# lrjconan/LanczosNetwork

Measured on AMD Instinct MI355X. Metric: molecules/sec LanczosNet forward, QM8 batch=1024, higher is better.
Workload: dtype f32; 1 GPU; QM8 LanczosNet batch=1024/GPU, N<=32 dense L (tile N=26), K=20, fp32, 7x128 layers, 1xMI355X per rank; step = [pack L + batch plan + Lanczos + tridiagonal eigensolver (Ritz pairs)] (one launch) + spectral gains + fused forward; global_batch=1024, parallelism=dp1 (batch shards, async score all-gather per step)

## Files before the change

include/lanczosnet_hip.h:

```cpp
#ifndef LANCZOSNET_HIP_H_
#define LANCZOSNET_HIP_H_

#include <stdint.h>

#ifdef __cplusplus
extern "C" {
#endif

#define LNZ_ABI_VERSION 7
#define LNZ_OK 0
#define LNZ_EINVAL (-1)
#define LNZ_ELAUNCH (-2)
#define LNZ_ENOTSUP (-3)

#define LNZ_TILE 32
#define LNZ_MAX_CHANNELS 32
#define LNZ_STRIP_SUB 6
#define LNZ_STRIP_INTS 80
#define LNZ_STRIP_MAX_B 2048
#define LNZ_RARE_DEBUG_INTS 512

typedef void* lnz_stream_t;

int lnz_abi_version(void);
// ... 154 lines not shown
int lnz_pack_rows_k8(const float* W, int rows, int cols, int64_t ld, float* Wp,
                     lnz_stream_t stream);
int lnz_pack_rows_k8_split(const float* W, int rows, int cols, int64_t ld, float* Wp,
                           lnz_stream_t stream);
int64_t lnz_pack_fold_weights_size(int num_layer, int din0, int dhid);
int lnz_pack_fold_weights(const float* Wp, const int64_t* w_off_host, int num_layer, int din0, int dhid,
                          int n_short, int n_long, int n_edge, float* Wf, lnz_stream_t stream);
int lnz_pack_bias_rows(const float* bias, int rows, float* bp, lnz_stream_t stream);
int lnz_pack_laplacian(const float* L, int64_t stride_b, int64_t stride_r, int64_t stride_c,
                       int64_t stride_ch, int B, int N, int C, float* Lp, lnz_stream_t stream);
int lnz_pack_laplacian_ident(const float* L, int64_t stride_b, int64_t stride_r, int64_t stride_c,
                             int64_t stride_ch, int B, int N, int C, float* Lp, uint32_t* ident,
                             lnz_stream_t stream);

int64_t lnz_spectral_mlp_pack_size(int S);
int lnz_pack_spectral_mlp(const float* W0, const float* b0, const float* W2, const float* b2,
                          const float* W4, const float* b4, const float* W6, const float* b6,
                          int S, float* pack, lnz_stream_t stream);
int lnz_pack_spectral_mlp_layers(const float* const* ptrs, int num_layer, int S, float* pack,
                                 lnz_stream_t stream);
int lnz_spectral_gains(const float* D, int B, int K, const int32_t* dist_host, int S,
                       int num_layer, int kind, const float* mlp_pack, float* G,
                       lnz_stream_t stream);
int lnz_spectral_gains_rows(const float* D, int B, int K, const int32_t* dist_host, int S,
                            int num_layer, int kind, const float* mlp_pack, const int32_t* rows,
                            const int32_t* n_rows, float* G, lnz_stream_t stream);

int lnz_spectral_mlp_grad_floats(int S);
int lnz_spectral_mlp_grad_parts(int n_rows_max, int num_layer, int n_cu);
int lnz_spectral_mlp_grad(const float* D, int B, int K, const int32_t* dist_host, int S,
// ... 266 lines not shown
```

lanczosnet_amd/_lib.py:

```python
import ctypes as C
import os

_HERE = os.path.dirname(os.path.abspath(__file__))
LIB_PATH = os.environ.get('LANCZOSNET_HIP_LIB') or os.path.join(_HERE, 'csrc', 'liblanczosnet_hip.so')

LNZ_OK, LNZ_EINVAL, LNZ_ELAUNCH, LNZ_ENOTSUP = 0, -1, -2, -3
ABI_VERSION = 7


class LnzError(RuntimeError):
  def __init__(self, code, msg):
    super().__init__('lanczosnet_hip error %d: %s' % (code, msg))
    self.code = code


class NotSupported(LnzError, NotImplementedError):
  pass


class ForwardArgs(C.Structure):
  _fields_ = [
      ('B', C.c_int32), ('N', C.c_int32), ('K', C.c_int32),
      ('num_layer', C.c_int32),
      ('din0', C.c_int32), ('dhid', C.c_int32), ('dout', C.c_int32),
# ... 91 lines not shown
    'lnz_pack_fold_weights_size': (C.c_int64, [_I, _I, _I]),
    'lnz_pack_fold_weights': (C.c_int, [_P, C.POINTER(C.c_int64), _I, _I, _I, _I, _I, _I, _P, _P]),
    'lnz_pack_bias_rows': (C.c_int, [_P, _I, _P, _P]),
    'lnz_pack_laplacian': (C.c_int, [_P, _L, _L, _L, _L, _I, _I, _I, _P, _P]),
    'lnz_collate_qm8': (C.c_int, [_P, _P, _P, _P, _P, _P, _L, _I, _I, _I, _I, _P, _P, _P, _P, _P, _P]),
    'lnz_plan_wg_cap': (C.c_int, [_I, _I]),
    'lnz_pack_laplacian_plan': (C.c_int, [_P, _L, _L, _L, _L, _I, _I, _I, _P, _P, _I, _I, _P, _P, _I, _P, _P, _P, _P, _P, _P]),
    'lnz_pack_laplacian_ident': (C.c_int, [_P, _L, _L, _L, _L, _I, _I, _I, _P, _P, _P]),
    'lnz_prepare_batch_prev_gains': (C.c_int, [_P, _L, _L, _L, _L, _I, _I, _I, _P, _P, _P, _I, _I, _P, _P, _I, _P, _P, _P, _P, _P, _P, _I, _P, _P, C.POINTER(C.c_int32), _I, _I, _P, _P, _P, _P, _P]),
    'lnz_prepare_batch': (C.c_int, [_P, _L, _L, _L, _L, _I, _I, _I, _P, _P, _P, _I, _I, _P, _P, _I, _P, _P, _P, _P, _P, _P, _P, _P, _P]),
    'lnz_plan_batch': (C.c_int, [_P, _I, _I, _I, _I, _P, _P, _I, _P, _P, _P, _P, _P]),
    'lnz_plan_strips': (C.c_int, [_P, _I, _I, _I, _P, _P, _P]),
    'lnz_strip_cap': (C.c_int, [_I]),
    'lnz_plan_tiles': (C.c_int, [_P, _I, _I, _I, _I, _P, _P, _P]),
    'lnz_spectral_mlp_pack_size': (C.c_int64, [_I]),
    'lnz_pack_spectral_mlp': (C.c_int, [_P] * 8 + [_I, _P, _P]),
    'lnz_pack_spectral_mlp_layers': (C.c_int, [_P, _I, _I, _P, _P]),
    'lnz_spectral_mlp_grad_parts': (C.c_int, [_I, _I, _I]),
    'lnz_spectral_gains_rows_split': (C.c_int, [_P, _I, _I, _P, _I, _I, _I, _P, _P, _P, _P, _P, _L, _P]),
    'lnz_spectral_gains_rows_split_to': (C.c_int, [_P, _I, _I, _P, _I, _I, _I, _P, _P, _P, _P, _P, _P, _L, _P]),
    'lnz_split_laplacian_pack': (C.c_int, [_P, _L, _P]),
    'lnz_split_laplacian_pack_to': (C.c_int, [_P, _L, _P, _P]),
    'lnz_spectral_mlp_grad_floats': (C.c_int, [_I]),
    'lnz_embedding_grad': (C.c_int, [_P, _I, _I, _P, _L, _L, _I, _I, _I, _P, _P]),
    'lnz_spectral_mlp_grad': (C.c_int, [_P, _I, _I, _P, _I, _I, _P, _P, _P, _P, _I, _P, _P]),
    'lnz_spectral_gains': (C.c_int, [_P, _I, _I, C.POINTER(C.c_int32), _I, _I, _I, _P, _P, _P]),
    'lnz_spectral_gains_rows': (C.c_int, [_P, _I, _I, C.POINTER(C.c_int32), _I, _I, _I, _P, _P, _P, _P, _P]),
    'lnz_lanczosnet_input_grad': (C.c_int, [C.POINTER(ForwardArgs), _P]),
    'lnz_lanczosnet_messages': (C.c_int, [C.POINTER(ForwardArgs), _P]),
    'lnz_lanczosnet_gain_grad': (C.c_int, [C.POINTER(ForwardArgs), _P]),
# ... 87 lines not shown
```

lanczosnet_amd/csrc/gains_body.hpp:

```cpp
#pragma once
#include "common.hpp"

namespace lnz_gains {

constexpr int HID = 128;
constexpr int HT = HID / 32;
constexpr int SMAX = 16;
constexpr int OFF_W0 = 0;
constexpr int OFF_B0 = OFF_W0 + HT * 8 * 64;
constexpr int OFF_B2 = OFF_B0 + HT * 1024;
constexpr int OFF_B4 = OFF_B2 + HT * 1024;
constexpr int OFF_B6 = OFF_B4 + HT * 1024;
constexpr int OFF_W2 = OFF_B6 + 1024;
constexpr int OFF_W4 = OFF_W2 + HT * 16 * 256;
constexpr int OFF_W6 = OFF_W4 + HT * 16 * 256;
#ifndef LNZ_GAINS_RING
#define LNZ_GAINS_RING 8
#endif
#ifndef LNZ_GAINS_DIST
#define LNZ_GAINS_DIST (LNZ_GAINS_RING - 2)
#endif
constexpr int RING = LNZ_GAINS_RING;
constexpr int PACK_SIZE = OFF_W6 + 16 * 256 + RING * 256;
constexpr int NSTEP = 2 * HT * 16 + 16;

struct DistArr {
  int32_t v[SMAX];
};

__device__ inline float powi(float x, int p) {
  double base = (double)x, acc = 1.0;
  int e = p < 0 ? -p : p;
  while (e) {
    if (e & 1) acc *= base;
    base *= base;
    e >>= 1;
  }
  return (float)(p < 0 ? 1.0 / acc : acc);
}

__device__ inline f32x16 load_bias_frag(const float* __restrict__ bp, int lane) {
  const float4* p = reinterpret_cast<const float4*>(bp) + lane * 4;
  f32x16 acc;
// ... 39 lines not shown
#pragma unroll
    for (int t = 0; t < RT; ++t) acc1[t] = lnz::mfma32(a.y, Hin[t][ti][4 * g + 1], acc1[t]);
#pragma unroll
    for (int t = 0; t < RT; ++t) acc[t] = lnz::mfma32(a.z, Hin[t][ti][4 * g + 2], acc[t]);
#pragma unroll
    for (int t = 0; t < RT; ++t) acc1[t] = lnz::mfma32(a.w, Hin[t][ti][4 * g + 3], acc1[t]);
    __builtin_amdgcn_sched_barrier(0);
  }
#pragma unroll
  for (int t = 0; t < RT; ++t) {
#pragma unroll
    for (int i = 0; i < 16; ++i) res[t][i] = acc[t][i] + acc1[t][i];
  }
}

template <int RT>
__device__ __forceinline__ void gains_mlp_tiles(const float* __restrict__ D, const int (&row)[RT],
                                                const bool (&valid)[RT], const int l,
                                                const int lane, int B, int K, const DistArr& dist,
                                                int S, const float* __restrict__ mlp_pack,
                                                float* __restrict__ G) {
  const int hh = lane >> 5;
  const float* pk = mlp_pack + (int64_t)l * PACK_SIZE;
#ifdef LNZ_GAINS_PROBE_STAGGER
  for (int i = 0; i < (int)((blockIdx.x & (LNZ_GAINS_PROBE_STAGGER_N - 1)) * LNZ_GAINS_PROBE_STAGGER); ++i)
    __builtin_amdgcn_s_sleep(16);
#endif

  const float4* __restrict__ wstream = reinterpret_cast<const float4*>(pk + OFF_W2) + lane;
  float4 ring[RING];
#pragma unroll
  for (int f = 0; f < LNZ_GAINS_DIST; ++f) ring[f] = wstream[f * 64];

  const int steps0 = S < 8 ? S : 8;
  f32x16 h1[RT][HT], h2[RT][HT];
  {
    float w0[HT][8];
#pragma unroll
    for (int ot = 0; ot < HT; ++ot) {
#pragma unroll
      for (int t = 0; t < 8; ++t) w0[ot][t] = pk[OFF_W0 + (ot * 8 + t) * 64 + lane];
    }
#pragma unroll
    for (int rt = 0; rt < RT; ++rt) {
      const float dval = valid[rt] ? D[row[rt]] : 0.0f;
      float feat[8];
#pragma unroll
      for (int t = 0; t < 8; ++t) {
#ifdef LNZ_GAINS_PROBE_NOPOW
        float lo = t < S ? dval : 0.0f;
        float hi = (8 + t) < S ? dval : 0.0f;
// ... 16 lines not shown
  }
  f32x16 res[RT];
#define LNZ_DENSE(F0, IN, OUT, OT, BOFF)                                   \
  {                                                                        \
    const f32x16 bb = load_bias_frag(pk + (BOFF), lane);                   \
    dense_tile<F0, RT>(wstream, ring, IN, res);                            \
    _Pragma("unroll") for (int rt = 0; rt < RT; ++rt) OUT[rt][OT] = relu_bias16(res[rt], bb); \
  }
  LNZ_DENSE(0, h1, h2, 0, OFF_B2 + 0 * 1024)
  LNZ_DENSE(16, h1, h2, 1, OFF_B2 + 1 * 1024)
  LNZ_DENSE(32, h1, h2, 2, OFF_B2 + 2 * 1024)
  LNZ_DENSE(48, h1, h2, 3, OFF_B2 + 3 * 1024)
  LNZ_DENSE(64, h2, h1, 0, OFF_B4 + 0 * 1024)
  LNZ_DENSE(80, h2, h1, 1, OFF_B4 + 1 * 1024)
  LNZ_DENSE(96, h2, h1, 2, OFF_B4 + 2 * 1024)
  LNZ_DENSE(112, h2, h1, 3, OFF_B4 + 3 * 1024)
#undef LNZ_DENSE
  {
    const f32x16 b6 = load_bias_frag(pk + OFF_B6, lane);
    dense_tile<128, RT>(wstream, ring, h1, res);
#pragma unroll
    for (int rt = 0; rt < RT; ++rt) {
      if (valid[rt]) {
        const int b = row[rt] / K, k = row[rt] - b * K;
        float* Gb = G + (((int64_t)l * B + b) * S) * K + k;
#pragma unroll
        for (int r = 0; r < 16; ++r) {
          int sidx = lnz::cd_row(r, hh);
          if (sidx < S) Gb[(int64_t)sidx * K] = res[rt][r] + b6[r];
        }
      }
    }
  }
}

__device__ __forceinline__ void gains_mlp_tile(const float* __restrict__ D, const int row,
                                               const bool valid, const int l, const int lane,
                                               int B, int K, const DistArr& dist, int S,
                                               const float* __restrict__ mlp_pack,
                                               float* __restrict__ G) {
  const int rows1[1] = {row};
  const bool valid1[1] = {valid};
  gains_mlp_tiles<1>(D, rows1, valid1, l, lane, B, K, dist, S, mlp_pack, G);
}

}
```

lanczosnet_amd/csrc/lanczos_ritz.hip:

```cpp
#include "common.hpp"
#include "prep.hpp"
#include "gains_body.hpp"
#include "tql2.hpp"

namespace {

using lnz::kEpsF64;
using lnz::rcp_nr;
using lnz::readlane_f64;

constexpr double kBreakdownTol = 1e-8;

struct Ritz32Smem {
  static constexpr int LD = 34;
  double* Qt;
  double* za;
  double* zb;
  double* ca;
  double* cb;
  double* dd;
  double* Dw;
  double2* de;
  int* perm;
  float* sgn;
// ... 801 lines not shown
    if (threadIdx.x >= 64) return;
    lanczos_ritz32_body(L, sb, sr, sc, n_nodes, N, K, D, V, info, blk - 2, threadIdx.x,
                        ritz32_view(ubuf, N));
  } else {
    pack_laplacian_body(L, sb, sr, sc, sch, N, C, Lp, reinterpret_cast<float*>(ubuf), blk - 2 - B,
                        ident);
  }
}

static size_t prep_lds_bytes(int N, int C) {
  size_t lds = (size_t)N * N * C * sizeof(float);
  lds = lds > ritz32_lds_bytes(N) ? lds : ritz32_lds_bytes(N);
  return lds > (size_t)kStripScratch ? lds : (size_t)kStripScratch;
}

__global__ __launch_bounds__(256, 2) void prepare_batch_gains_kernel(
    const float* __restrict__ L, int64_t sb, int64_t sr, int64_t sc, int64_t sch, int N, int C,
    float4* __restrict__ Lp, const uint8_t* __restrict__ mask, int B, int n_cu, int allow_pairs,
    int wg_cap, int32_t* __restrict__ plan, int32_t* __restrict__ n_wg, int K,
    int32_t* __restrict__ gain_rows, int32_t* __restrict__ n_gain_rows,
    const int32_t* __restrict__ n_nodes, float* __restrict__ D, float* __restrict__ V,
    lnz_gains::DistArr dist, int S, int num_layer,
    const float* __restrict__ mlp_pack, float* __restrict__ G, uint32_t* __restrict__ ident,
    int n_cons, const float* __restrict__ Dg, const int32_t* __restrict__ rows_g,
    const int32_t* __restrict__ n_rows_g, int Bg, int32_t* __restrict__ strips,
    int32_t* __restrict__ n_strips) {
  extern __shared__ __attribute__((aligned(16))) unsigned char ubuf[];
  const Ritz32Smem sm = ritz32_view(ubuf, N);
  float* tile = reinterpret_cast<float*>(ubuf);
  const int blk = blockIdx.x;
// ... 9 lines not shown
    lanczos_ritz32_body(L, sb, sr, sc, n_nodes, N, K, D, V, nullptr, blk - 2, threadIdx.x, sm);
  } else {
    const int p = blk - B - 2;
    if (p >= n_cons) {
      pack_laplacian_body(L, sb, sr, sc, sch, N, C, Lp, tile, p - n_cons, ident);
      return;
    }
    const int lane = threadIdx.x & 63;
    const int gw = p * 4 + (threadIdx.x >> 6);
    const int t = gw / num_layer, l = gw - t * num_layer;
    const int R = *n_rows_g;
    if (32 * t >= R) return;
    const int idx = 32 * t + (lane & 31);
    const bool valid = idx < R;
    const int row = valid ? rows_g[idx] : 0;
    lnz_gains::gains_mlp_tile(Dg, row, valid, l, lane, Bg, K, dist, S, mlp_pack, G);
  }
}

}

extern "C" int lnz_prepare_batch(const float* L, int64_t stride_b, int64_t stride_r,
                                 int64_t stride_c, int64_t stride_ch, int B, int N, int C,
                                 float* Lp, const uint8_t* mask, const int32_t* n_nodes, int n_cu,
                                 int allow_pairs, int32_t* plan, int32_t* n_wg, int K,
                                 int32_t* gain_rows, int32_t* n_gain_rows, float* D, float* V,
                                 int32_t* info, uint32_t* ident, int32_t* strips,
                                 int32_t* n_strips, lnz_stream_t stream) {
  LNZ_REQUIRE(L && mask && n_nodes && plan && n_wg && D && V && B > 0 && C > 0 &&
                  C <= LNZ_MAX_CHANNELS && n_cu > 0 && K > 0,
              LNZ_EINVAL, "lnz_prepare_batch: bad arguments (B=%d C=%d K=%d)", B, C, K);
// ... 24 lines not shown
                  D_prev && rows_prev && n_rows_prev && dist_host && mlp_pack && G_prev && B > 0 &&
                  B_prev > 0 && C > 0 && C <= LNZ_MAX_CHANNELS && n_cu > 0 && K > 0 && num_layer > 0,
              LNZ_EINVAL, "lnz_prepare_batch_prev_gains: bad arguments (B=%d C=%d K=%d)", B, C, K);
  LNZ_REQUIRE(N > 0 && N <= LNZ_TILE, LNZ_ENOTSUP, "lnz_prepare_batch_prev_gains: N=%d > %d", N,
              LNZ_TILE);
  LNZ_REQUIRE(S >= 1 && S <= lnz_gains::SMAX, LNZ_ENOTSUP, "lnz_prepare_batch_prev_gains: S=%d", S);
  const size_t tile = (size_t)N * N * C * sizeof(float);
  LNZ_REQUIRE(tile <= 40 * 1024, LNZ_ENOTSUP,
              "lnz_prepare_batch_prev_gains: N*N*C*4 = %zu B exceeds the 40 KiB staging tile", tile);
  lnz_gains::DistArr dist;
  for (int i = 0; i < lnz_gains::SMAX; ++i) dist.v[i] = i < S ? dist_host[i] : 0;
  const int64_t tiles = ((int64_t)B_prev * K + 31) / 32;
  const int64_t n_cons = (tiles * num_layer + 3) / 4;
  const int64_t grid = 2 * (int64_t)B + 2 + n_cons;
  LNZ_REQUIRE(grid < (1ll << 31), LNZ_ENOTSUP, "lnz_prepare_batch_prev_gains: batch too large");
  hipLaunchKernelGGL(prepare_batch_gains_kernel, dim3((unsigned)grid), dim3(256),
                     prep_lds_bytes(N, C), (hipStream_t)stream, L, stride_b, stride_r, stride_c, stride_ch, N, C,
                     (float4*)Lp, mask, B, n_cu, allow_pairs, lnz_plan_wg_cap(B, n_cu), plan, n_wg,
                     K, gain_rows, n_gain_rows, n_nodes, D, V, dist, S, num_layer, mlp_pack, G_prev,
                     ident, (int)n_cons, D_prev, rows_prev, n_rows_prev, B_prev,
                     (strips && n_strips) ? strips : nullptr, n_strips);
  return lnz::check_launch("lnz_prepare_batch_prev_gains");
}

int lnz_launch_ritz_wg(const float* A, int64_t stride_b, int64_t stride_r, int64_t stride_c,
                       const int32_t* n_nodes, int B, int N, int K, float* D, float* V,
                       int32_t* info, void* workspace, int64_t workspace_bytes, int flags,
                       hipStream_t s);

extern "C" int lnz_lanczos_ritz(const float* A, int64_t stride_b, int64_t stride_r,
                                int64_t stride_c, const int32_t* n_nodes, int B, int N, int K,
// ... 120 lines not shown
```

lanczosnet_amd/csrc/spectral_gains.hip:

```cpp
#include "common.hpp"
#include "gains_body.hpp"
#include "split_pack.hpp"
#include <stdlib.h>

namespace {

using namespace lnz_gains;

__global__ void pack_w0_kernel(const float* __restrict__ W0, int S, float* __restrict__ out) {
  int idx = blockIdx.x * blockDim.x + threadIdx.x;
  if (idx >= HT * 8 * 64) return;
  int lane = idx & 63, t = (idx >> 6) & 7, ot = idx >> 9;
  int f = 8 * (lane >> 5) + t;
  out[idx] = f < S ? W0[(32 * ot + (lane & 31)) * S + f] : 0.0f;
}

struct SplitRide {
  const float4* pack;
  float4* dst;
  int64_t n4;
  int main_x;
};
__device__ __forceinline__ bool ride_along(const SplitRide& r, const int lane) {
  if (!r.pack || (int)blockIdx.x < r.main_x) return false;
  const int64_t chunk = (int64_t)(blockIdx.x - r.main_x) * gridDim.y + blockIdx.y;
  if (chunk * lnz::kSplitChunk < r.n4) lnz::split_pack_chunk<64>(r.pack, r.dst, r.n4, chunk, lane);
  return true;
}

__global__ __launch_bounds__(64) void spectral_gains_mlp_kernel(
    const float* __restrict__ D, int R, int B, int K, DistArr dist, int S,
    const float* __restrict__ mlp_pack, const int32_t* __restrict__ rows,
    const int32_t* __restrict__ n_rows, float* __restrict__ G, const SplitRide ride) {
  const int lane = threadIdx.x;
  if (ride_along(ride, lane)) return;
  if (rows) R = *n_rows;
  if ((int)blockIdx.x * 32 >= R) return;
  const int idx = blockIdx.x * 32 + (lane & 31);
  const bool valid = idx < R;
  const int row = valid ? (rows ? rows[idx] : idx) : 0;
  gains_mlp_tile(D, row, valid, blockIdx.y, lane, B, K, dist, S, mlp_pack, G);
}

__global__ __launch_bounds__(64) void spectral_gains_mlp2_kernel(
    const float* __restrict__ D, int R, int B, int K, DistArr dist, int S,
    const float* __restrict__ mlp_pack, const int32_t* __restrict__ rows,
    const int32_t* __restrict__ n_rows, float* __restrict__ G, const SplitRide ride) {
  const int lane = threadIdx.x;
  if (ride_along(ride, lane)) return;
  if (rows) R = *n_rows;
  if ((int)blockIdx.x * 64 >= R) return;
  int row[2];
  bool valid[2];
#pragma unroll
  for (int t = 0; t < 2; ++t) {
    const int idx = blockIdx.x * 64 + 32 * t + (lane & 31);
    valid[t] = idx < R;
    row[t] = valid[t] ? (rows ? rows[idx] : idx) : 0;
  }
  gains_mlp_tiles<2>(D, row, valid, blockIdx.y, lane, B, K, dist, S, mlp_pack, G);
}

__global__ void spectral_gains_pow_kernel(const float* __restrict__ D, int B, int K, DistArr dist,
                                          int S, int num_layer, float* __restrict__ G) {
  int64_t idx = (int64_t)blockIdx.x * blockDim.x + threadIdx.x;
  int64_t total = (int64_t)num_layer * B * S * K;
  if (idx >= total) return;
  int k = (int)(idx % K);
  int s = (int)((idx / K) % S);
  int b = (int)((idx / ((int64_t)K * S)) % B);
  G[idx] = powi(D[(int64_t)b * K + k], dist.v[s]);
}

}

extern "C" int64_t lnz_spectral_mlp_pack_size(int S) {
  (void)S;
  return PACK_SIZE;
}

extern "C" int lnz_pack_spectral_mlp(const float* W0, const float* b0, const float* W2,
                                     const float* b2, const float* W4, const float* b4,
                                     const float* W6, const float* b6, int S, float* pack,
                                     lnz_stream_t stream) {
  LNZ_REQUIRE(S >= 1 && S <= SMAX, LNZ_ENOTSUP, "lnz_pack_spectral_mlp: S=%d not in 1..%d", S,
              SMAX);
  LNZ_REQUIRE(W0 && b0 && W2 && b2 && W4 && b4 && W6 && b6 && pack, LNZ_EINVAL,
              "lnz_pack_spectral_mlp: null pointer");
  hipLaunchKernelGGL(pack_w0_kernel, dim3((HT * 8 * 64 + 255) / 256), dim3(256), 0,
                     (hipStream_t)stream, W0, S, pack + OFF_W0);
  int rc = lnz::check_launch("lnz_pack_spectral_mlp(W0)");
  if (rc) return rc;
  if ((rc = lnz_pack_bias_rows(b0, HID, pack + OFF_B0, stream))) return rc;
  if ((rc = lnz_pack_rows_k8(W2, HID, HID, HID, pack + OFF_W2, stream))) return rc;
  if ((rc = lnz_pack_bias_rows(b2, HID, pack + OFF_B2, stream))) return rc;
  if ((rc = lnz_pack_rows_k8(W4, HID, HID, HID, pack + OFF_W4, stream))) return rc;
  if ((rc = lnz_pack_bias_rows(b4, HID, pack + OFF_B4, stream))) return rc;
  if ((rc = lnz_pack_rows_k8(W6, S, HID, HID, pack + OFF_W6, stream))) return rc;
  if ((rc = lnz_pack_bias_rows(b6, S, pack + OFF_B6, stream))) return rc;
  return LNZ_OK;
}

struct MlpLayerPtrs {
  const float* p[16][8];
};

__device__ inline float rows_k8_elem(const float* __restrict__ W, int rows, int cols, int ld,
                                     int Q, int f) {
  const int idx4 = f >> 2, u = f & 3;
  const int lane = idx4 & 63, q = (idx4 >> 6) % Q, rt = (idx4 >> 6) / Q;
  const int row = 32 * rt + (lane & 31), col = 8 * q + 4 * (lane >> 5) + u;
  return (row < rows && col < cols) ? W[(int64_t)row * ld + col] : 0.0f;
}

__device__ inline float bias_rows_elem(const float* __restrict__ b, int rows, int f) {
// ... 14 lines not shown
    v = feat < S ? pl[0][(32 * ot + (lane & 31)) * S + feat] : 0.0f;
  } else if (f < OFF_B2) {
    v = bias_rows_elem(pl[1], HID, f - OFF_B0);
  } else if (f < OFF_B4) {
    v = bias_rows_elem(pl[3], HID, f - OFF_B2);
  } else if (f < OFF_B6) {
    v = bias_rows_elem(pl[5], HID, f - OFF_B4);
  } else if (f < OFF_W2) {
    v = bias_rows_elem(pl[7], S, f - OFF_B6);
  } else if (f < OFF_W4) {
    v = rows_k8_elem(pl[2], HID, HID, HID, HID / 8, f - OFF_W2);
  } else if (f < OFF_W6) {
    v = rows_k8_elem(pl[4], HID, HID, HID, HID / 8, f - OFF_W4);
  } else if (f < OFF_W6 + 16 * 256) {
    v = rows_k8_elem(pl[6], S, HID, HID, HID / 8, f - OFF_W6);
  }
  pack[(int64_t)l * PACK_SIZE + f] = v;
}

extern "C" int lnz_pack_spectral_mlp_layers(const float* const* ptrs, int num_layer, int S,
                                            float* pack, lnz_stream_t stream) {
  LNZ_REQUIRE(S >= 1 && S <= SMAX, LNZ_ENOTSUP, "lnz_pack_spectral_mlp_layers: S=%d not in 1..%d",
              S, SMAX);
  LNZ_REQUIRE(ptrs && pack && num_layer >= 1 && num_layer <= 16, LNZ_EINVAL,
              "lnz_pack_spectral_mlp_layers: bad arguments (L=%d)", num_layer);
  MlpLayerPtrs mp;
  for (int l = 0; l < 16; ++l)
    for (int i = 0; i < 8; ++i) {
      mp.p[l][i] = l < num_layer ? ptrs[l * 8 + i] : nullptr;
      LNZ_REQUIRE(l >= num_layer || mp.p[l][i], LNZ_EINVAL,
// ... 22 lines not shown
  hipStream_t s = (hipStream_t)stream;
  if (kind == 0) {
    LNZ_REQUIRE(mlp_pack, LNZ_EINVAL, "lnz_spectral_gains: kind=MLP needs mlp_pack");
    int R = B * K;
    static const int forced = [] {
      const char* e = getenv("LNZ_GAINS_TILES");
      return e ? atoi(e) : 0;
    }();
    const bool two = forced ? forced == 2 : (int64_t)((R + 31) / 32) * num_layer >= 2048;
    SplitRide ride = {reinterpret_cast<const float4*>(Lp_split), reinterpret_cast<float4*>(Lp_dst), lp_floats / 4,
                      (R + (two ? 63 : 31)) / (two ? 64 : 32)};
    const int64_t chunks = Lp_split ? (ride.n4 + lnz::kSplitChunk - 1) / lnz::kSplitChunk : 0;
    const int64_t extra_x = (chunks + num_layer - 1) / num_layer;
    LNZ_REQUIRE(ride.main_x + extra_x < (1ll << 31), LNZ_ENOTSUP, "lnz_spectral_gains_rows_split: pack too large");
    dim3 grid((unsigned)(ride.main_x + extra_x), num_layer);
    if (two) {
      hipLaunchKernelGGL(spectral_gains_mlp2_kernel, grid, dim3(64), 0, s, D, R, B, K, dist, S,
                         mlp_pack, rows, n_rows, G, ride);
    } else {
      hipLaunchKernelGGL(spectral_gains_mlp_kernel, grid, dim3(64), 0, s, D, R, B, K, dist, S,
                         mlp_pack, rows, n_rows, G, ride);
    }
  } else {
    int64_t total = (int64_t)num_layer * B * S * K;
    hipLaunchKernelGGL(spectral_gains_pow_kernel, dim3((int)((total + 255) / 256)), dim3(256), 0,
                       s, D, B, K, dist, S, num_layer, G);
  }
  return lnz::check_launch("lnz_spectral_gains");
}

extern "C" int lnz_spectral_gains_rows_split(const float* D, int B, int K, const int32_t* dist_host,
                                             int S, int num_layer, int kind, const float* mlp_pack,
                                             const int32_t* rows, const int32_t* n_rows, float* G,
                                             float* Lp_split, int64_t lp_floats, lnz_stream_t stream) {
  return lnz_spectral_gains_rows_split_to(D, B, K, dist_host, S, num_layer, kind, mlp_pack, rows, n_rows, G,
                                          Lp_split, reinterpret_cast<uint16_t*>(Lp_split), lp_floats, stream);
}
// ... 16 lines not shown
```

lanczosnet_amd/csrc/torch_ext_abi.inc:

```

void raw_laplacian_l4(const c10::optional<Tensor>& adjs, const c10::optional<Tensor>& n_nodes, int64_t B, int64_t N, int64_t E, const c10::optional<Tensor>& L) {
  const Tensor* first_ = first_defined({(adjs.has_value() ? &*adjs : nullptr), (n_nodes.has_value() ? &*n_nodes : nullptr), (L.has_value() ? &*L : nullptr)});
  c10::OptionalDeviceGuard guard_;
  if (first_) guard_.reset_device(first_->device());
  check(lnz_laplacian_l4((const float*)raw_ptr(adjs, at::kFloat, "adjs"), (const int32_t*)raw_ptr(n_nodes, at::kInt, "n_nodes"), (int)B, (int)N, (int)E, (float*)raw_ptr(L, at::kFloat, "L"), cur_stream()), "laplacian_l4");
}
void raw_laplacian(const c10::optional<Tensor>& adjs, const c10::optional<Tensor>& n_nodes, int64_t B, int64_t N, int64_t E, int64_t kind, double alpha, const c10::optional<Tensor>& L) {
  const Tensor* first_ = first_defined({(adjs.has_value() ? &*adjs : nullptr), (n_nodes.has_value() ? &*n_nodes : nullptr), (L.has_value() ? &*L : nullptr)});
  c10::OptionalDeviceGuard guard_;
  if (first_) guard_.reset_device(first_->device());
  check(lnz_laplacian((const float*)raw_ptr(adjs, at::kFloat, "adjs"), (const int32_t*)raw_ptr(n_nodes, at::kInt, "n_nodes"), (int)B, (int)N, (int)E, (int)kind, (double)alpha, (float*)raw_ptr(L, at::kFloat, "L"), cur_stream()), "laplacian");
}
void raw_lanczos_ritz(const c10::optional<Tensor>& A, int64_t stride_b, int64_t stride_r, int64_t stride_c, const c10::optional<Tensor>& n_nodes, int64_t B, int64_t N, int64_t K, const c10::optional<Tensor>& D, const c10::optional<Tensor>& V, const c10::optional<Tensor>& info) {
  const Tensor* first_ = first_defined({(A.has_value() ? &*A : nullptr), (n_nodes.has_value() ? &*n_nodes : nullptr), (D.has_value() ? &*D : nullptr), (V.has_value() ? &*V : nullptr), (info.has_value() ? &*info : nullptr)});
  c10::OptionalDeviceGuard guard_;
  if (first_) guard_.reset_device(first_->device());
  check(lnz_lanczos_ritz((const float*)raw_ptr(A, at::kFloat, "A"), (int64_t)stride_b, (int64_t)stride_r, (int64_t)stride_c, (const int32_t*)raw_ptr(n_nodes, at::kInt, "n_nodes"), (int)B, (int)N, (int)K, (float*)raw_ptr(D, at::kFloat, "D"), (float*)raw_ptr(V, at::kFloat, "V"), (int32_t*)raw_ptr(info, at::kInt, "info"), cur_stream()), "lanczos_ritz");
}
int64_t raw_lanczos_ritz_workspace_bytes(int64_t B, int64_t N) {
  return (int64_t)lnz_lanczos_ritz_workspace_bytes((int)B, (int)N);
}
void raw_lanczos_ritz_ws(const c10::optional<Tensor>& A, int64_t stride_b, int64_t stride_r, int64_t stride_c, const c10::optional<Tensor>& n_nodes, int64_t B, int64_t N, int64_t K, const c10::optional<Tensor>& D, const c10::optional<Tensor>& V, const c10::optional<Tensor>& info, const c10::optional<Tensor>& workspace, int64_t workspace_bytes, int64_t flags) {
  const Tensor* first_ = first_defined({(A.has_value() ? &*A : nullptr), (n_nodes.has_value() ? &*n_nodes : nullptr), (D.has_value() ? &*D : nullptr), (V.has_value() ? &*V : nullptr), (info.has_value() ? &*info : nullptr), (workspace.has_value() ? &*workspace : nullptr)});
  c10::OptionalDeviceGuard guard_;
// ... 257 lines not shown
}
void raw_pack_laplacian(const c10::optional<Tensor>& L, int64_t stride_b, int64_t stride_r, int64_t stride_c, int64_t stride_ch, int64_t B, int64_t N, int64_t C, const c10::optional<Tensor>& Lp) {
  const Tensor* first_ = first_defined({(L.has_value() ? &*L : nullptr), (Lp.has_value() ? &*Lp : nullptr)});
  c10::OptionalDeviceGuard guard_;
  if (first_) guard_.reset_device(first_->device());
  check(lnz_pack_laplacian((const float*)raw_ptr(L, at::kFloat, "L"), (int64_t)stride_b, (int64_t)stride_r, (int64_t)stride_c, (int64_t)stride_ch, (int)B, (int)N, (int)C, (float*)raw_ptr(Lp, at::kFloat, "Lp"), cur_stream()), "pack_laplacian");
}
void raw_pack_laplacian_ident(const c10::optional<Tensor>& L, int64_t stride_b, int64_t stride_r, int64_t stride_c, int64_t stride_ch, int64_t B, int64_t N, int64_t C, const c10::optional<Tensor>& Lp, const c10::optional<Tensor>& ident) {
  const Tensor* first_ = first_defined({(L.has_value() ? &*L : nullptr), (Lp.has_value() ? &*Lp : nullptr), (ident.has_value() ? &*ident : nullptr)});
  c10::OptionalDeviceGuard guard_;
  if (first_) guard_.reset_device(first_->device());
  check(lnz_pack_laplacian_ident((const float*)raw_ptr(L, at::kFloat, "L"), (int64_t)stride_b, (int64_t)stride_r, (int64_t)stride_c, (int64_t)stride_ch, (int)B, (int)N, (int)C, (float*)raw_ptr(Lp, at::kFloat, "Lp"), (uint32_t*)raw_ptr(ident, at::kInt, "ident"), cur_stream()), "pack_laplacian_ident");
}
int64_t raw_spectral_mlp_pack_size(int64_t S) {
  return (int64_t)lnz_spectral_mlp_pack_size((int)S);
}
void raw_pack_spectral_mlp(const c10::optional<Tensor>& W0, const c10::optional<Tensor>& b0, const c10::optional<Tensor>& W2, const c10::optional<Tensor>& b2, const c10::optional<Tensor>& W4, const c10::optional<Tensor>& b4, const c10::optional<Tensor>& W6, const c10::optional<Tensor>& b6, int64_t S, const c10::optional<Tensor>& pack) {
  const Tensor* first_ = first_defined({(W0.has_value() ? &*W0 : nullptr), (b0.has_value() ? &*b0 : nullptr), (W2.has_value() ? &*W2 : nullptr), (b2.has_value() ? &*b2 : nullptr), (W4.has_value() ? &*W4 : nullptr), (b4.has_value() ? &*b4 : nullptr), (W6.has_value() ? &*W6 : nullptr), (b6.has_value() ? &*b6 : nullptr), (pack.has_value() ? &*pack : nullptr)});
  c10::OptionalDeviceGuard guard_;
  if (first_) guard_.reset_device(first_->device());
  check(lnz_pack_spectral_mlp((const float*)raw_ptr(W0, at::kFloat, "W0"), (const float*)raw_ptr(b0, at::kFloat, "b0"), (const float*)raw_ptr(W2, at::kFloat, "W2"), (const float*)raw_ptr(b2, at::kFloat, "b2"), (const float*)raw_ptr(W4, at::kFloat, "W4"), (const float*)raw_ptr(b4, at::kFloat, "b4"), (const float*)raw_ptr(W6, at::kFloat, "W6"), (const float*)raw_ptr(b6, at::kFloat, "b6"), (int)S, (float*)raw_ptr(pack, at::kFloat, "pack"), cur_stream()), "pack_spectral_mlp");
}
void raw_pack_spectral_mlp_layers(at::TensorList ptrs, int64_t num_layer, int64_t S, const c10::optional<Tensor>& pack) {
  std::vector<const float*> ptrs_v;
  for (const Tensor& t_ : ptrs) {
    need(t_, at::kFloat, "ptrs[i]");
    ptrs_v.push_back(t_.data_ptr<float>());
  }
  const Tensor* first_ = first_defined({(ptrs.empty() ? nullptr : &ptrs[0]), (pack.has_value() ? &*pack : nullptr)});
  c10::OptionalDeviceGuard guard_;
// ... 413 lines not shown
  m.def("raw_lanczos_ritz_kstep_wide_edges_workspace_bytes(int B, int N, int M, int row_cap, int conv_row_cap) -> int"); \
  m.def("raw_lanczos_ritz_kstep_wide_edges(Tensor? edges, int n_edges, Tensor? edge_off, Tensor? n_nodes, int B, int N, int M, int K, int row_cap, int row_order, Tensor(a!)? workspace, int workspace_bytes, Tensor(b!)? D, Tensor(c!)? V, Tensor(d!)? info, Tensor(e!)? fallback, Tensor(f!)? conv_entries, Tensor(g!)? conv_values, Tensor(h!)? conv_counts, int conv_row_cap, int conv_order, Tensor(i!)? conv_flags, Tensor(j!)? status) -> ()"); \
  m.def("raw_laplacian_l4_edges_image_workspace_bytes(int B, int N, int conv_row_cap) -> int"); \
  m.def("raw_laplacian_l4_edges_image(Tensor? edges, int n_edges, Tensor? edge_off, Tensor? n_nodes, int B, int N, Tensor(a!)? workspace, int workspace_bytes, Tensor(b!)? conv_entries, Tensor(c!)? conv_values, Tensor(d!)? conv_counts, int conv_row_cap, int conv_order, Tensor(e!)? conv_flags, Tensor(f!)? status) -> ()"); \
  m.def("raw_laplacian_l4_typed_edges_images_workspace_bytes(int B, int N, int num_edge_type, int conv_row_cap) -> int"); \
  m.def("raw_laplacian_l4_typed_edges_images(Tensor? edges, Tensor? edge_type, int n_edges, Tensor? edge_off, Tensor? n_nodes, int B, int N, int num_edge_type, Tensor(a!)? workspace, int workspace_bytes, Tensor(b!)? conv_entries, Tensor(c!)? conv_values, Tensor(d!)? conv_counts, int conv_row_cap, Tensor(e!)? conv_flags, Tensor(f!)? status) -> ()"); \
  m.def("raw_packed_rows_k8_size(int rows, int cols) -> int"); \
  m.def("raw_pack_rows_k8(Tensor? W, int rows, int cols, int ld, Tensor(a!)? Wp) -> ()"); \
  m.def("raw_pack_rows_k8_split(Tensor? W, int rows, int cols, int ld, Tensor(a!)? Wp) -> ()"); \
  m.def("raw_pack_fold_weights_size(int num_layer, int din0, int dhid) -> int"); \
  m.def("raw_pack_fold_weights(Tensor? Wp, int[]? w_off_host, int num_layer, int din0, int dhid, int n_short, int n_long, int n_edge, Tensor(a!)? Wf) -> ()"); \
  m.def("raw_pack_bias_rows(Tensor? bias, int rows, Tensor(a!)? bp) -> ()"); \
  m.def("raw_pack_laplacian(Tensor? L, int stride_b, int stride_r, int stride_c, int stride_ch, int B, int N, int C, Tensor(a!)? Lp) -> ()"); \
  m.def("raw_pack_laplacian_ident(Tensor? L, int stride_b, int stride_r, int stride_c, int stride_ch, int B, int N, int C, Tensor(a!)? Lp, Tensor(b!)? ident) -> ()"); \
  m.def("raw_spectral_mlp_pack_size(int S) -> int"); \
  m.def("raw_pack_spectral_mlp(Tensor? W0, Tensor? b0, Tensor? W2, Tensor? b2, Tensor? W4, Tensor? b4, Tensor? W6, Tensor? b6, int S, Tensor(a!)? pack) -> ()"); \
  m.def("raw_pack_spectral_mlp_layers(Tensor[] ptrs, int num_layer, int S, Tensor(a!)? pack) -> ()"); \
  m.def("raw_spectral_gains(Tensor? D, int B, int K, int[]? dist_host, int S, int num_layer, int kind, Tensor? mlp_pack, Tensor(a!)? G) -> ()"); \
  m.def("raw_spectral_gains_rows(Tensor? D, int B, int K, int[]? dist_host, int S, int num_layer, int kind, Tensor? mlp_pack, Tensor? rows, Tensor? n_rows, Tensor(a!)? G) -> ()"); \
  m.def("raw_spectral_mlp_grad_floats(int S) -> int"); \
  m.def("raw_spectral_mlp_grad_parts(int n_rows_max, int num_layer, int n_cu) -> int"); \
  m.def("raw_spectral_mlp_grad(Tensor? D, int B, int K, int[]? dist_host, int S, int num_layer, Tensor? rows, Tensor? n_rows, Tensor? dG, Tensor[] ptrs, int parts, Tensor(a!)? partials) -> ()"); \
  m.def("raw_embedding_grad(Tensor? ids, int B, int N, Tensor? dx, int mol_stride, int row_stride, int width, int num_atom, int chunks, Tensor(a!)? partials) -> ()"); \
  m.def("raw_spectral_gains_rows_split(Tensor? D, int B, int K, int[]? dist_host, int S, int num_layer, int kind, Tensor? mlp_pack, Tensor? rows, Tensor? n_rows, Tensor(a!)? G, Tensor(b!)? Lp_split, int lp_floats) -> ()"); \
  m.def("raw_split_laplacian_pack(Tensor(a!)? Lp, int n_floats) -> ()"); \
  m.def("raw_spectral_gains_rows_split_to(Tensor? D, int B, int K, int[]? dist_host, int S, int num_layer, int kind, Tensor? mlp_pack, Tensor? rows, Tensor? n_rows, Tensor(a!)? G, Tensor? Lp_split, Tensor(b!)? Lp_dst, int lp_floats) -> ()"); \
  m.def("raw_split_laplacian_pack_to(Tensor? Lp, int n_floats, Tensor(a!)? dst) -> ()"); \
  m.def("raw_plan_wg_cap(int B, int n_cu) -> int"); \
  m.def("raw_plan_tiles(Tensor? mask, int B, int N, int n_cu, int allow_pairs, Tensor(a!)? plan, Tensor(b!)? n_wg) -> ()"); \
  m.def("raw_plan_batch(Tensor? mask, int B, int N, int n_cu, int allow_pairs, Tensor(a!)? plan, Tensor(b!)? n_wg, int K, Tensor(c!)? gain_rows, Tensor(d!)? n_gain_rows, Tensor(e!)? strips, Tensor(f!)? n_strips) -> ()"); \
// ... 150 lines not shown

#define LNZ_RAW_IMPLS_HOST(m) \
  m.impl("raw_lanczos_ritz_workspace_bytes", raw_lanczos_ritz_workspace_bytes); \
  m.impl("raw_large_nk", raw_large_nk); \
  m.impl("raw_lanczos_ritz_large_workspace_bytes", raw_lanczos_ritz_large_workspace_bytes); \
  m.impl("raw_lanczos_ritz_kstep_workspace_bytes", raw_lanczos_ritz_kstep_workspace_bytes); \
  m.impl("raw_lanczos_ritz_kstep_wide_workspace_bytes", raw_lanczos_ritz_kstep_wide_workspace_bytes); \
  m.impl("raw_sym_eigh_topk_workspace_bytes", raw_sym_eigh_topk_workspace_bytes); \
  m.impl("raw_lanczos_ritz_kstep_edges_workspace_bytes", raw_lanczos_ritz_kstep_edges_workspace_bytes); \
  m.impl("raw_lanczos_ritz_kstep_wide_edges_workspace_bytes", raw_lanczos_ritz_kstep_wide_edges_workspace_bytes); \
  m.impl("raw_laplacian_l4_edges_image_workspace_bytes", raw_laplacian_l4_edges_image_workspace_bytes); \
  m.impl("raw_laplacian_l4_typed_edges_images_workspace_bytes", raw_laplacian_l4_typed_edges_images_workspace_bytes); \
  m.impl("raw_packed_rows_k8_size", raw_packed_rows_k8_size); \
  m.impl("raw_pack_fold_weights_size", raw_pack_fold_weights_size); \
  m.impl("raw_spectral_mlp_pack_size", raw_spectral_mlp_pack_size); \
  m.impl("raw_spectral_mlp_grad_floats", raw_spectral_mlp_grad_floats); \
  m.impl("raw_spectral_mlp_grad_parts", raw_spectral_mlp_grad_parts); \
  m.impl("raw_plan_wg_cap", raw_plan_wg_cap); \
  m.impl("raw_strip_cap", raw_strip_cap); \
  m.impl("raw_head_backward_workspace_floats", raw_head_backward_workspace_floats); \
  m.impl("raw_midgraph_workspace_floats", raw_midgraph_workspace_floats); \
  m.impl("raw_midgraph_head_grad_workspace_floats", raw_midgraph_head_grad_workspace_floats); \
  m.impl("raw_midgraph_project_workspace_floats", raw_midgraph_project_workspace_floats); \
  m.impl("raw_forward_args_size", raw_forward_args_size); \
  m.impl("raw_ada_laplacian_f64_state_doubles", raw_ada_laplacian_f64_state_doubles); \
  m.impl("raw_ada_lanczos_f64_workspace_doubles", raw_ada_lanczos_f64_workspace_doubles); \
  m.impl("raw_f16x3_linear_splits", raw_f16x3_linear_splits); \
  m.impl("raw_f32_linear_splits", raw_f32_linear_splits); \
  m.impl("raw_f32_linear_workspace_floats", raw_f32_linear_workspace_floats); \
  m.impl("raw_gat_attention_backward_workspace_floats", raw_gat_attention_backward_workspace_floats); \
// ... 4 lines not shown
```

Measured before the change: 1.493 million molecules/s.

## Use compact weight packing and 4x4 MFMA for spectral gains MLP ends

Adds a compact packed form for the spectral MLP's first and last layers. The first layer now uses only as many MFMA steps as needed when S<=8. The last linear layer is computed with 4x4x1 MFMAs over groups of four outputs instead of a full 32-wide dense tile, and stores results straight to G. This cuts wasted MFMA work and weight streaming when the output width S is small. The trade-offs are a larger pack buffer, an env-var switch that is on by default, and more complex lane-swap logic.

```diff
diff --git a/include/lanczosnet_hip.h b/include/lanczosnet_hip.h
--- a/include/lanczosnet_hip.h
+++ b/include/lanczosnet_hip.h
@@ -192,6 +192,7 @@
                              lnz_stream_t stream);
 
 int64_t lnz_spectral_mlp_pack_size(int S);
+int64_t lnz_spectral_mlp_pack_source(int S, int64_t f);
 int lnz_pack_spectral_mlp(const float* W0, const float* b0, const float* W2, const float* b2,
                           const float* W4, const float* b4, const float* W6, const float* b6,
                           int S, float* pack, lnz_stream_t stream);
diff --git a/lanczosnet_amd/_lib.py b/lanczosnet_amd/_lib.py
--- a/lanczosnet_amd/_lib.py
+++ b/lanczosnet_amd/_lib.py
@@ -129,6 +129,7 @@
     'lnz_strip_cap': (C.c_int, [_I]),
     'lnz_plan_tiles': (C.c_int, [_P, _I, _I, _I, _I, _P, _P, _P]),
     'lnz_spectral_mlp_pack_size': (C.c_int64, [_I]),
+    'lnz_spectral_mlp_pack_source': (C.c_int64, [_I, _L]),
     'lnz_pack_spectral_mlp': (C.c_int, [_P] * 8 + [_I, _P, _P]),
     'lnz_pack_spectral_mlp_layers': (C.c_int, [_P, _I, _I, _P, _P]),
     'lnz_spectral_mlp_grad_parts': (C.c_int, [_I, _I, _I]),
diff --git a/lanczosnet_amd/csrc/gains_body.hpp b/lanczosnet_amd/csrc/gains_body.hpp
--- a/lanczosnet_amd/csrc/gains_body.hpp
+++ b/lanczosnet_amd/csrc/gains_body.hpp
@@ -1,5 +1,7 @@
 #pragma once
 #include "common.hpp"
+#include <stdlib.h>
+#include <type_traits>
 
 namespace lnz_gains {
 
@@ -21,12 +23,42 @@
 #define LNZ_GAINS_DIST (LNZ_GAINS_RING - 2)
 #endif
 constexpr int RING = LNZ_GAINS_RING;
-constexpr int PACK_SIZE = OFF_W6 + 16 * 256 + RING * 256;
+constexpr int PACK_V1 = OFF_W6 + 16 * 256 + RING * 256;
+constexpr int OFF_W0C = PACK_V1;
+constexpr int OFF_W6C = OFF_W0C + HT * 4 * 64;
+constexpr int PACK_SIZE = OFF_W6C + (SMAX / 4) * 8 * 64;
 constexpr int NSTEP = 2 * HT * 16 + 16;
 
 struct DistArr {
   int32_t v[SMAX];
 };
+
+inline bool compact_form() {
+  static const bool on = [] {
+    const char* e = getenv("LNZ_GAINS_COMPACT");
+    return e ? atoi(e) != 0 : true;
+  }();
+  return on;
+}
+
+__host__ __device__ inline int64_t compact_source(int S, int f, int* tensor) {
+  *tensor = -1;
+  if (f < OFF_W6C) {
+    const int g = f - OFF_W0C;
+    const int lane = g & 63, u = (g >> 6) & 3, ot = g >> 8;
+    const int feat = 2 * u + (lane >> 5);
+    if (feat >= S) return 0;
+    *tensor = 0;
+    return (int64_t)(32 * ot + (lane & 31)) * S + feat;
+  }
+  const int g = f - OFF_W6C;
+  const int lane = g & 63, v = (g >> 6) & 7, grp = g >> 9;
+  const int blk = lane >> 2, row = 4 * grp + (lane & 3);
+  const int j = blk & 7, q = 2 * v + (blk >> 3);
+  if (row >= S) return 0;
+  *tensor = 6;
+  return (int64_t)row * HID + 8 * q + (((j & 1) << 2) | (j & 2) | (j >> 2));
+}
 
 __device__ inline float powi(float x, int p) {
   double base = (double)x, acc = 1.0;
@@ -96,7 +128,75 @@
   }
 }
 
-template <int RT>
+template <int ABID>
+__device__ inline f32x4 mfma4(float a, float b, f32x4 c) {
+  return __builtin_amdgcn_mfma_f32_4x4x1f32(a, b, c, 4, ABID, 0);
+}
+
+template <int Q, int NG, bool SWAP>
+__device__ inline void last_linear_step(const float (&wa)[2][8], f32x16 (&lo)[HT], f32x16 (&hi)[HT],
+                                        f32x4 (&acc)[NG], f32x4 (&acc1)[NG]) {
+  constexpr int ti = Q >> 2, g = Q & 3, v = Q >> 1, A0 = 8 * (Q & 1);
+  if constexpr (SWAP) {
+#pragma unroll
+    for (int r = 4 * g; r < 4 * g + 4; ++r) {
+      const auto sw = __builtin_amdgcn_permlane32_swap(__float_as_uint(lo[ti][r]),
+                                                       __float_as_uint(hi[ti][r]), false, false);
+      lo[ti][r] = __uint_as_float(sw[0]);
+      hi[ti][r] = __uint_as_float(sw[1]);
+    }
+  }
+#pragma unroll
+  for (int n = 0; n < NG; ++n) acc[n] = mfma4<A0 + 0>(wa[n][v], lo[ti][4 * g + 0], acc[n]);
+#pragma unroll
+  for (int n = 0; n < NG; ++n) acc1[n] = mfma4<A0 + 4>(wa[n][v], lo[ti][4 * g + 1], acc1[n]);
+#pragma unroll
+  for (int n = 0; n < NG; ++n) acc[n] = mfma4<A0 + 1>(wa[n][v], hi[ti][4 * g + 0], acc[n]);
+#pragma unroll
+  for (int n = 0; n < NG; ++n) acc1[n] = mfma4<A0 + 5>(wa[n][v], hi[ti][4 * g + 1], acc1[n]);
+#pragma unroll
+  for (int n = 0; n < NG; ++n) acc[n] = mfma4<A0 + 2>(wa[n][v], lo[ti][4 * g + 2], acc[n]);
+#pragma unroll
+  for (int n = 0; n < NG; ++n) acc1[n] = mfma4<A0 + 6>(wa[n][v], lo[ti][4 * g + 3], acc1[n]);
+#pragma unroll
+  for (int n = 0; n < NG; ++n) acc[n] = mfma4<A0 + 3>(wa[n][v], hi[ti][4 * g + 2], acc[n]);
+#pragma unroll
+  for (int n = 0; n < NG; ++n) acc1[n] = mfma4<A0 + 7>(wa[n][v], hi[ti][4 * g + 3], acc1[n]);
+  if constexpr (Q + 1 < 16) last_linear_step<Q + 1, NG, SWAP>(wa, lo, hi, acc, acc1);
+}
+
+__device__ inline void load_last_weights(const float* __restrict__ wl, float (&wa)[2][8]) {
+#pragma unroll
+  for (int n = 0; n < 2; ++n) {
+#pragma unroll
+    for (int v = 0; v < 8; ++v) wa[n][v] = wl[(n * 8 + v) * 64];
+  }
+}
+
+template <int NG, bool SWAP>
+__device__ inline void last_linear_groups(const float (&wa)[2][8], f32x16 (&lo)[HT],
+                                          f32x16 (&hi)[HT], f32x4 (&out)[NG]) {
+  f32x4 acc[NG], acc1[NG];
+#pragma unroll
+  for (int n = 0; n < NG; ++n) {
+    acc[n] = f32x4{0.0f, 0.0f, 0.0f, 0.0f};
+    acc1[n] = f32x4{0.0f, 0.0f, 0.0f, 0.0f};
+  }
+  last_linear_step<0, NG, SWAP>(wa, lo, hi, acc, acc1);
+#pragma unroll
+  for (int n = 0; n < NG; ++n) out[n] = acc[n] + acc1[n];
+}
+
+__device__ inline void store_group(const f32x4 v, const int grp, const int S, const int64_t K,
+                                   const float* __restrict__ b6p, float* __restrict__ Gb) {
+#pragma unroll
+  for (int i = 0; i < 4; ++i) {
+    const int s = 4 * grp + i;
+    if (s < S) Gb[s * K] = v[i] + b6p[((s >> 2) & 1) * 512 + (s & 3) + 4 * (s >> 3)];
+  }
+}
+
+template <int RT, bool COMPACT>
 __device__ __forceinline__ void gains_mlp_tiles(const float* __restrict__ D, const int (&row)[RT],
                                                 const bool (&valid)[RT], const int l,
                                                 const int lane, int B, int K, const DistArr& dist,
@@ -116,7 +216,34 @@
 
   const int steps0 = S < 8 ? S : 8;
   f32x16 h1[RT][HT], h2[RT][HT];
-  {
+  if (COMPACT && S <= 8) {
+    const int steps = (S + 1) >> 1;
+    float w0[HT][4];
+#pragma unroll
+    for (int ot = 0; ot < HT; ++ot) {
+#pragma unroll
+      for (int u = 0; u < 4; ++u) w0[ot][u] = pk[OFF_W0C + (ot * 4 + u) * 64 + lane];
+    }
+#pragma unroll
+    for (int rt = 0; rt < RT; ++rt) {
+      const float dval = valid[rt] ? D[row[rt]] : 0.0f;
+      float feat[4];
+#pragma unroll
+      for (int u = 0; u < 4; ++u) {
+        const int p = hh ? dist.v[2 * u + 1] : dist.v[2 * u];
+        feat[u] = 2 * u + hh < S ? powi(dval, p) : 0.0f;
+      }
+#pragma unroll
+      for (int ot = 0; ot < HT; ++ot) {
+        f32x16 acc = lnz::splat16(0.0f);
+#pragma unroll
+        for (int u = 0; u < 4; ++u) {
+          if (u < steps) acc = lnz::mfma32(w0[ot][u], feat[u], acc);
+        }
+        h1[rt][ot] = relu_bias16(acc, load_bias_frag(pk + OFF_B0 + ot * 1024, lane));
+      }
+    }
+  } else {
     float w0[HT][8];
 #pragma unroll
     for (int ot = 0; ot < HT; ++ot) {
@@ -163,9 +290,54 @@
   LNZ_DENSE(64, h2, h1, 0, OFF_B4 + 0 * 1024)
   LNZ_DENSE(80, h2, h1, 1, OFF_B4 + 1 * 1024)
   LNZ_DENSE(96, h2, h1, 2, OFF_B4 + 2 * 1024)
+  const float* wl = pk + OFF_W6C + lane;
+  float wa0[2][8];
+  if constexpr (COMPACT) load_last_weights(wl, wa0);
   LNZ_DENSE(112, h2, h1, 3, OFF_B4 + 3 * 1024)
 #undef LNZ_DENSE
-  {
+  if constexpr (COMPACT) {
+#pragma unroll
+    for (int n = 0; n < 2; ++n) {
+#pragma unroll
+      for (int v = 0; v < 8; ++v) asm volatile("" : "+v"(wa0[n][v]));
+    }
+  }
+  if constexpr (COMPACT) {
+    static_assert(RT <= 2, "one lane half per tile");
+    f32x16 self[HT];
+    if constexpr (RT == 1) {
+#pragma unroll
+      for (int ti = 0; ti < HT; ++ti) self[ti] = h1[0][ti];
+    }
+    f32x16(&lo)[HT] = h1[0];
+    f32x16(&hi)[HT] = *(RT == 1 ? &self : &h1[RT - 1]);
+    const int mine = RT == 2 ? hh : 0;
+    const bool ok = RT == 2 ? valid[mine] : (valid[0] && hh == 0);
+    const int myrow = row[mine];
+    const int b = myrow / K, k = myrow - b * K;
+    float* Gb = G + (((int64_t)l * B + b) * S) * K + k;
+    const int ng = (S + 3) >> 2;
+    auto pass = [&](auto swap, const float (&wa)[2][8], const int g0) {
+      if (g0 + 1 < ng) {
+        f32x4 o[2];
+        last_linear_groups<2, decltype(swap)::value>(wa, lo, hi, o);
+        if (ok) {
+          store_group(o[0], g0, S, K, pk + OFF_B6, Gb);
+          store_group(o[1], g0 + 1, S, K, pk + OFF_B6, Gb);
+        }
+      } else {
+        f32x4 o[1];
+        last_linear_groups<1, decltype(swap)::value>(wa, lo, hi, o);
+        if (ok) store_group(o[0], g0, S, K, pk + OFF_B6, Gb);
+      }
+    };
+    pass(std::true_type{}, wa0, 0);
+    if (ng > 2) {
+      float wa2[2][8];
+      load_last_weights(wl + 2 * 512, wa2);
+      pass(std::false_type{}, wa2, 2);
+    }
+  } else {
     const f32x16 b6 = load_bias_frag(pk + OFF_B6, lane);
     dense_tile<128, RT>(wstream, ring, h1, res);
 #pragma unroll
@@ -183,6 +355,7 @@
   }
 }
 
+template <bool COMPACT>
 __device__ __forceinline__ void gains_mlp_tile(const float* __restrict__ D, const int row,
                                                const bool valid, const int l, const int lane,
                                                int B, int K, const DistArr& dist, int S,
@@ -190,7 +363,7 @@
                                                float* __restrict__ G) {
   const int rows1[1] = {row};
   const bool valid1[1] = {valid};
-  gains_mlp_tiles<1>(D, rows1, valid1, l, lane, B, K, dist, S, mlp_pack, G);
-}
-
-}
+  gains_mlp_tiles<1, COMPACT>(D, rows1, valid1, l, lane, B, K, dist, S, mlp_pack, G);
+}
+
+}
diff --git a/lanczosnet_amd/csrc/lanczos_ritz.hip b/lanczosnet_amd/csrc/lanczos_ritz.hip
--- a/lanczosnet_amd/csrc/lanczos_ritz.hip
+++ b/lanczosnet_amd/csrc/lanczos_ritz.hip
@@ -839,6 +839,7 @@
   return lds > (size_t)kStripScratch ? lds : (size_t)kStripScratch;
 }
 
+template <bool COMPACT>
 __global__ __launch_bounds__(256, 2) void prepare_batch_gains_kernel(
     const float* __restrict__ L, int64_t sb, int64_t sr, int64_t sc, int64_t sch, int N, int C,
     float4* __restrict__ Lp, const uint8_t* __restrict__ mask, int B, int n_cu, int allow_pairs,
@@ -878,7 +879,7 @@
     const int idx = 32 * t + (lane & 31);
     const bool valid = idx < R;
     const int row = valid ? rows_g[idx] : 0;
-    lnz_gains::gains_mlp_tile(Dg, row, valid, l, lane, Bg, K, dist, S, mlp_pack, G);
+    lnz_gains::gains_mlp_tile<COMPACT>(Dg, row, valid, l, lane, Bg, K, dist, S, mlp_pack, G);
   }
 }
 
@@ -933,7 +934,8 @@
   const int64_t n_cons = (tiles * num_layer + 3) / 4;
   const int64_t grid = 2 * (int64_t)B + 2 + n_cons;
   LNZ_REQUIRE(grid < (1ll << 31), LNZ_ENOTSUP, "lnz_prepare_batch_prev_gains: batch too large");
-  hipLaunchKernelGGL(prepare_batch_gains_kernel, dim3((unsigned)grid), dim3(256),
+  auto kernel = lnz_gains::compact_form() ? prepare_batch_gains_kernel<true> : prepare_batch_gains_kernel<false>;
+  hipLaunchKernelGGL(kernel, dim3((unsigned)grid), dim3(256),
                      prep_lds_bytes(N, C), (hipStream_t)stream, L, stride_b, stride_r, stride_c, stride_ch, N, C,
                      (float4*)Lp, mask, B, n_cu, allow_pairs, lnz_plan_wg_cap(B, n_cu), plan, n_wg,
                      K, gain_rows, n_gain_rows, n_nodes, D, V, dist, S, num_layer, mlp_pack, G_prev,
diff --git a/lanczosnet_amd/csrc/spectral_gains.hip b/lanczosnet_amd/csrc/spectral_gains.hip
--- a/lanczosnet_amd/csrc/spectral_gains.hip
+++ b/lanczosnet_amd/csrc/spectral_gains.hip
@@ -13,6 +13,19 @@
   int lane = idx & 63, t = (idx >> 6) & 7, ot = idx >> 9;
   int f = 8 * (lane >> 5) + t;
   out[idx] = f < S ? W0[(32 * ot + (lane & 31)) * S + f] : 0.0f;
+}
+
+__device__ inline float compact_elem(const float* __restrict__ W0, const float* __restrict__ W6,
+                                     int S, int f) {
+  int tensor;
+  const int64_t src = compact_source(S, f, &tensor);
+  return tensor == 0 ? W0[src] : tensor == 6 ? W6[src] : 0.0f;
+}
+
+__global__ void pack_compact_kernel(const float* __restrict__ W0, const float* __restrict__ W6,
+                                    int S, float* __restrict__ pack) {
+  const int f = OFF_W0C + blockIdx.x * blockDim.x + threadIdx.x;
+  if (f < PACK_SIZE) pack[f] = compact_elem(W0, W6, S, f);
 }
 
 struct SplitRide {
@@ -28,6 +41,7 @@
   return true;
 }
 
+template <bool COMPACT>
 __global__ __launch_bounds__(64) void spectral_gains_mlp_kernel(
     const float* __restrict__ D, int R, int B, int K, DistArr dist, int S,
     const float* __restrict__ mlp_pack, const int32_t* __restrict__ rows,
@@ -39,9 +53,10 @@
   const int idx = blockIdx.x * 32 + (lane & 31);
   const bool valid = idx < R;
   const int row = valid ? (rows ? rows[idx] : idx) : 0;
-  gains_mlp_tile(D, row, valid, blockIdx.y, lane, B, K, dist, S, mlp_pack, G);
-}
-
+  gains_mlp_tile<COMPACT>(D, row, valid, blockIdx.y, lane, B, K, dist, S, mlp_pack, G);
+}
+
+template <bool COMPACT>
 __global__ __launch_bounds__(64) void spectral_gains_mlp2_kernel(
     const float* __restrict__ D, int R, int B, int K, DistArr dist, int S,
     const float* __restrict__ mlp_pack, const int32_t* __restrict__ rows,
@@ -58,7 +73,7 @@
     valid[t] = idx < R;
     row[t] = valid[t] ? (rows ? rows[idx] : idx) : 0;
   }
-  gains_mlp_tiles<2>(D, row, valid, blockIdx.y, lane, B, K, dist, S, mlp_pack, G);
+  gains_mlp_tiles<2, COMPACT>(D, row, valid, blockIdx.y, lane, B, K, dist, S, mlp_pack, G);
 }
 
 __global__ void spectral_gains_pow_kernel(const float* __restrict__ D, int B, int K, DistArr dist,
@@ -77,6 +92,13 @@
 extern "C" int64_t lnz_spectral_mlp_pack_size(int S) {
   (void)S;
   return PACK_SIZE;
+}
+
+extern "C" int64_t lnz_spectral_mlp_pack_source(int S, int64_t f) {
+  if (S < 1 || S > SMAX || f < OFF_W0C || f >= PACK_SIZE) return -2;
+  int tensor;
+  const int64_t src = compact_source(S, (int)f, &tensor);
+  return tensor < 0 ? -1 : ((int64_t)(tensor == 6) << 32) + src;
 }
 
 extern "C" int lnz_pack_spectral_mlp(const float* W0, const float* b0, const float* W2,
@@ -98,7 +120,9 @@
   if ((rc = lnz_pack_bias_rows(b4, HID, pack + OFF_B4, stream))) return rc;
   if ((rc = lnz_pack_rows_k8(W6, S, HID, HID, pack + OFF_W6, stream))) return rc;
   if ((rc = lnz_pack_bias_rows(b6, S, pack + OFF_B6, stream))) return rc;
-  return LNZ_OK;
+  hipLaunchKernelGGL(pack_compact_kernel, dim3((PACK_SIZE - OFF_W0C + 255) / 256), dim3(256), 0,
+                     (hipStream_t)stream, W0, W6, S, pack);
+  return lnz::check_launch("lnz_pack_spectral_mlp(compact)");
 }
 
 struct MlpLayerPtrs {
@@ -143,6 +167,8 @@
     v = rows_k8_elem(pl[4], HID, HID, HID, HID / 8, f - OFF_W4);
   } else if (f < OFF_W6 + 16 * 256) {
     v = rows_k8_elem(pl[6], S, HID, HID, HID / 8, f - OFF_W6);
+  } else if (f >= OFF_W0C) {
+    v = compact_elem(pl[0], pl[6], S, f);
   }
   pack[(int64_t)l * PACK_SIZE + f] = v;
 }
@@ -195,13 +221,10 @@
     const int64_t extra_x = (chunks + num_layer - 1) / num_layer;
     LNZ_REQUIRE(ride.main_x + extra_x < (1ll << 31), LNZ_ENOTSUP, "lnz_spectral_gains_rows_split: pack too large");
     dim3 grid((unsigned)(ride.main_x + extra_x), num_layer);
-    if (two) {
-      hipLaunchKernelGGL(spectral_gains_mlp2_kernel, grid, dim3(64), 0, s, D, R, B, K, dist, S,
-                         mlp_pack, rows, n_rows, G, ride);
-    } else {
-      hipLaunchKernelGGL(spectral_gains_mlp_kernel, grid, dim3(64), 0, s, D, R, B, K, dist, S,
-                         mlp_pack, rows, n_rows, G, ride);
-    }
+    auto kernel = two ? (compact_form() ? spectral_gains_mlp2_kernel<true> : spectral_gains_mlp2_kernel<false>)
+                      : (compact_form() ? spectral_gains_mlp_kernel<true> : spectral_gains_mlp_kernel<false>);
+    hipLaunchKernelGGL(kernel, grid, dim3(64), 0, s, D, R, B, K, dist, S, mlp_pack, rows, n_rows, G,
+                       ride);
   } else {
     int64_t total = (int64_t)num_layer * B * S * K;
     hipLaunchKernelGGL(spectral_gains_pow_kernel, dim3((int)((total + 255) / 256)), dim3(256), 0,
diff --git a/lanczosnet_amd/csrc/torch_ext_abi.inc b/lanczosnet_amd/csrc/torch_ext_abi.inc
--- a/lanczosnet_amd/csrc/torch_ext_abi.inc
+++ b/lanczosnet_amd/csrc/torch_ext_abi.inc
@@ -295,6 +295,9 @@
 }
 int64_t raw_spectral_mlp_pack_size(int64_t S) {
   return (int64_t)lnz_spectral_mlp_pack_size((int)S);
+}
+int64_t raw_spectral_mlp_pack_source(int64_t S, int64_t f) {
+  return (int64_t)lnz_spectral_mlp_pack_source((int)S, (int64_t)f);
 }
 void raw_pack_spectral_mlp(const c10::optional<Tensor>& W0, const c10::optional<Tensor>& b0, const c10::optional<Tensor>& W2, const c10::optional<Tensor>& b2, const c10::optional<Tensor>& W4, const c10::optional<Tensor>& b4, const c10::optional<Tensor>& W6, const c10::optional<Tensor>& b6, int64_t S, const c10::optional<Tensor>& pack) {
   const Tensor* first_ = first_defined({(W0.has_value() ? &*W0 : nullptr), (b0.has_value() ? &*b0 : nullptr), (W2.has_value() ? &*W2 : nullptr), (b2.has_value() ? &*b2 : nullptr), (W4.has_value() ? &*W4 : nullptr), (b4.has_value() ? &*b4 : nullptr), (W6.has_value() ? &*W6 : nullptr), (b6.has_value() ? &*b6 : nullptr), (pack.has_value() ? &*pack : nullptr)});
@@ -738,6 +741,7 @@
   m.def("raw_pack_laplacian(Tensor? L, int stride_b, int stride_r, int stride_c, int stride_ch, int B, int N, int C, Tensor(a!)? Lp) -> ()"); \
   m.def("raw_pack_laplacian_ident(Tensor? L, int stride_b, int stride_r, int stride_c, int stride_ch, int B, int N, int C, Tensor(a!)? Lp, Tensor(b!)? ident) -> ()"); \
   m.def("raw_spectral_mlp_pack_size(int S) -> int"); \
+  m.def("raw_spectral_mlp_pack_source(int S, int f) -> int"); \
   m.def("raw_pack_spectral_mlp(Tensor? W0, Tensor? b0, Tensor? W2, Tensor? b2, Tensor? W4, Tensor? b4, Tensor? W6, Tensor? b6, int S, Tensor(a!)? pack) -> ()"); \
   m.def("raw_pack_spectral_mlp_layers(Tensor[] ptrs, int num_layer, int S, Tensor(a!)? pack) -> ()"); \
   m.def("raw_spectral_gains(Tensor? D, int B, int K, int[]? dist_host, int S, int num_layer, int kind, Tensor? mlp_pack, Tensor(a!)? G) -> ()"); \
@@ -918,6 +922,7 @@
   m.impl("raw_packed_rows_k8_size", raw_packed_rows_k8_size); \
   m.impl("raw_pack_fold_weights_size", raw_pack_fold_weights_size); \
   m.impl("raw_spectral_mlp_pack_size", raw_spectral_mlp_pack_size); \
+  m.impl("raw_spectral_mlp_pack_source", raw_spectral_mlp_pack_source); \
   m.impl("raw_spectral_mlp_grad_floats", raw_spectral_mlp_grad_floats); \
   m.impl("raw_spectral_mlp_grad_parts", raw_spectral_mlp_grad_parts); \
   m.impl("raw_plan_wg_cap", raw_plan_wg_cap); \
```

New measurement: 1.511 million molecules/s (median of 6 runs). +1.2%, better.
